# wwood/CoverM

Measured on AMD Instinct MI355X. Metric: aligned reads/s through coverm contig (mean trimmed_mean covered_fraction variance), higher is better.
Workload: dtype i32 depth / u64 sums / f32 estimators

## Files before the change

### coverm_amd/csrc/covermhip.hip

```cpp
#include "pileup_kernels.hip.h"
#include "prep_lean.hip.h"
#include "genome_kernels.hip.h"
#include "sep_kernels.hip.h"
#include "ingest_kernels.hip.h"
#include "group_kernels.hip.h"
#include "sam_kernels.hip.h"
#include "gene_kernels.hip.h"
#include "depth_kernels.hip.h"
#include "depth_bins_kernels.hip.h"
#include "depth_regions_kernels.hip.h"

#include <algorithm>
#include <atomic>
#include <cstddef>
#include <chrono>
#include <cstdio>
#include <dlfcn.h>
#include <functional>
#include <sched.h>
#include <cstdlib>
#include <cstring>
#include <map>
#include <mutex>
#include <string>
// ... 185 lines not shown
        if (why == Reset::SAM_FILE) return;
        feed = ingplan::FeedState{}; launched = 0; copy_cleared = -1;
        key_lo = 0; key_hi = ingplan::KEY_END; search_first = false; open_end = false;
        span_lo = 0; tail_key = ~0ull;
        s_alloc = 0; for (double &x : s_part) x = 0;
        stats = cov_ingest_stats{};
    }
};

struct cov_session {
    cov_config cfg{};
    hipStream_t stream = nullptr;
    std::string err;
    int tile = 1024;
    bool use_fast = true;
    int chunk_tiles = 4;
    int prep_kernel = 0;
    int est_lanes = -1;
    int fast_tables = 1;
    int n_cus = 256;

    uint32_t n_targets = 0;
    std::vector<uint32_t> h_tlen;
    std::vector<uint32_t> h_tile_first;
    uint32_t n_tiles = 0;
    DevBuf<u32> d_tlen, d_tile_contig, d_tile_start;
    DevBuf<u32> d_tile_first, d_tcnt, d_fov, d_tscan, d_ttop;
    DevBuf<u32> d_slow_list;
    uint32_t tile_shift = 10;
    DevBuf<u32> d_cx_list, d_cx_cnt, d_cx_cur, d_cx_scan, d_cx_top;
    DevBuf<uint2> d_cx_runs;
    DevBuf<DevContig> d_ctg_scratch;
    DevBuf<int32_t> d_depth_all; DevBuf<u64> d_depth_off; bool depth_all_valid = false;
    DevBuf<DevInterval> d_iv; DevBuf<DevIntervalStats> d_ivst; DevBuf<unsigned long long> d_ivhist; uint64_t ivhist_total = 0;
    DevBuf<uint8_t> gr_code; DevBuf<u32> gr_mism, gr_trec, gr_pprim, gr_tids; DevBuf<int32_t> gr_ttid, gr_tpos; DevBuf<double> gr_ident, gr_tident, gr_ck;
    DevBuf<u64> gr_bcnt, gr_bmism, gr_pmism, gr_glob; DevBuf<gnrc::Interval> gr_iv; DevBuf<covgn::Out> gr_out; DevBuf<covgn::Bounds> gr_bounds;
    float gene_ms = 0.f; uint32_t gene_launches = 0;
    struct DepthRuns {
        DevBuf<int32_t> arena; DevBuf<u32> woff, mask, rank, sums, run_off; DevBuf<u64> doff, total; DevBuf<dprc::Run> runs;
        std::vector<u32> h_woff, h_run_off;
        u64 chunk_bases = dprc::DEFAULT_CHUNK_BASES;
        bool valid = false;
        u32 lo = 0, next = 0, launches = 0;
// ... 238 lines not shown
int pileup_occupancy(const cov_session *s, std::atomic<int> (&occ_dev)[64], const void *kern, size_t smem) {
    std::atomic<int> &occ_slot = occ_dev[(unsigned)s->cfg.device & 63u];
    int occ = occ_slot.load(std::memory_order_relaxed);
    if (!occ) {
        (void)hipFuncSetAttribute(kern, hipFuncAttributeMaxDynamicSharedMemorySize, (int)smem);
        int nb = 0;
        if (hipOccupancyMaxActiveBlocksPerMultiprocessor(&nb, kern, 256, smem) != hipSuccess || nb < 1) {
            (void)hipGetLastError();
            nb = (int)std::max<size_t>(1, std::min<size_t>(8, (160 * 1024) / smem));
        }
        occ = nb; occ_slot.store(nb, std::memory_order_relaxed);
    }
    return occ;
}
u32 pileup_grid(const cov_session *s, int occ, u32 n_tiles) {
    const u32 n_chunks = (n_tiles + (u32)s->chunk_tiles - 1) / (u32)s->chunk_tiles, wg_per_cu = 8u * (u32)occ;
    return std::max(1u, std::min((n_chunks + 3) / 4, (u32)s->n_cus * wg_per_cu));
}

template <bool H, int TABLES>
void launch_fast_v(cov_session *s, const PileupArgs &a, u32 n_tiles) {
    const auto kern = TABLES == 1 ? &k_pileup_fast<H> : &k_pileup_fast2t<H>;
    const size_t smem = pileup_fast_smem_bytes(H, TABLES == 1 ? FAST_HB : FAST_HB7, TABLES);
    static std::atomic<int> occ_dev[64];
    const int occ = pileup_occupancy(s, occ_dev, reinterpret_cast<const void *>(kern), smem);
    hipLaunchKernelGGL(kern, dim3(pileup_grid(s, occ, n_tiles)), dim3(256), smem, s->stream, a, n_tiles, (u32)s->chunk_tiles);
}
template <bool H>
void launch_fast_t(cov_session *s, const PileupArgs &a, u32 n_tiles) {
    if (s->fast_tables == 2) launch_fast_v<H, 2>(s, a, n_tiles);
    else launch_fast_v<H, 1>(s, a, n_tiles);
}

template <bool H, bool W>
void launch_stream_t(cov_session *s, const PileupArgs &a, u32 n_tiles, bool slow_list_only = false) {
    const size_t smem = pileup_stream_smem_bytes();
    static std::atomic<int> occ_dev[64];
    const int occ = pileup_occupancy(s, occ_dev, reinterpret_cast<const void *>(&k_pileup_stream<H, W>), smem);
    if (slow_list_only) {
        hipLaunchKernelGGL((k_pileup_stream<H, W>), dim3((u32)s->n_cus), dim3(256), smem, s->stream, a, 0u, 1u,
                           (const u32 *)s->d_slow_list.p, (const u32 *)&s->d_glob.p->n_slow);
// ... 110 lines not shown
        const char *mode = getenv("COVERM_PILEUP");
        if (mode && !strcmp(mode, "stream")) s->use_fast = false;
        s->tile = STREAM_TW;
        stamp("hipSetDevice");
        int cus = 0;
        if (hipDeviceGetAttribute(&cus, hipDeviceAttributeMultiprocessorCount, cfg->device) == hipSuccess && cus > 0) s->n_cus = cus;
        stamp("device attribute");
    }
    if (cfg->want & COV_WANT_INGEST) s->ing.prep = std::async(std::launch::async, [s] { return ingest_prepare_(s); });
    if (const char *el = getenv("COVERM_EST_LANES")) s->est_lanes = atoi(el) ? 1 : 0;
    if (const char *ft = getenv("COVERM_FAST_TABLES")) s->fast_tables = atoi(ft) == 2 ? 2 : 1;
    if (const char *pk = getenv("COVERM_PREP_KERNEL")) s->prep_kernel = atoi(pk) == 7 ? 7 : 0;
    if (const char *im = getenv("COVERM_IDENTITY")) s->id_mode = strcmp(im, "serial") ? 1 : 0;
    { long long v; if (covknob::get("store_cap_records", v) && v >= 1) s->cap_records = std::min<uint64_t>((uint64_t)v, 0xfffffff0ull); }
    { long long v; if (covknob::get("store_cap_cigar", v) && v >= 1) s->cap_cigar = std::min<uint64_t>((uint64_t)v, 0xfffffff0ull); }
    { long long v; if (covknob::get("pileup_chunk_tiles", v) && v >= 1 && v <= 64) s->chunk_tiles = (int)v; }
    { long long v; if (covknob::get("depth_chunk_bases", v) && v >= 4) s->dr.chunk_bases = (uint64_t)v; }
    e = hipEventCreateWithFlags(&s->ev_prep_done, hipEventDisableTiming);
    if (e == hipSuccess) e = hipEventCreateWithFlags(&s->ev_side_done, hipEventDisableTiming);
    if (e == hipSuccess) e = hipStreamCreateWithFlags(&s->stream, hipStreamNonBlocking);
    if (e != hipSuccess) { g_create_error = std::string("hipStreamCreate: ") + hipGetErrorString(e); (void)ingest_prep_wait(s); delete s; return COV_ERR_HIP; }
    stamp("streams and events");
    e = bind_result_block(s, 1);
    if (e != hipSuccess) { g_create_error = std::string("hipMalloc: ") + hipGetErrorString(e); cov_destroy(s); return COV_ERR_HIP; }
    stamp("first hipMalloc");
    *out = s;
    return COV_OK;
}

static void ingest_free_buffers(cov_session *s) {
    s->ing.free_buffers();
    for (auto &b : s->m_text) b.release();
    s->m_nl.release(); s->m_tab.release(); s->m_line_end.release(); s->m_cnt.release(); s->m_rec_idx.release(); s->m_cig_idx.release();
}

void cov_destroy(cov_session *s) {
    if (!s) return;
    (void)ingest_prep_wait(s);
    (void)hipSetDevice(s->cfg.device);
    if (s->stream) (void)hipStreamSynchronize(s->stream);
    s->d_tlen.release(); s->d_tile_contig.release(); s->d_tile_start.release(); s->d_mask.release();
    s->d_grow.release(); s->d_gtids.release(); s->d_gseg_genome.release(); s->d_gseg_start.release(); s->d_genomes.release(); s->d_ghist.release(); s->d_ghist_top.release(); s->d_order.release();
    s->d_sgid.release(); s->d_sblk.release(); s->d_sent_pos.release(); s->d_stop_last1.release(); s->d_stop_first.release(); s->d_scounts.release(); s->d_scode.release();
    s->d_stop_cnt.release(); s->d_stop_seg.release(); s->d_sent.release();
    s->d_gout.release(); if (s->h_gout) (void)hipHostFree(s->h_gout); s->h_gout = nullptr;
    s->d_tile_first.release(); s->d_tcnt.release(); s->d_fov.release(); s->d_tscan.release(); s->d_ttop.release(); s->d_slow_list.release();
    s->dr.release(); s->d_ctg_scratch.release(); s->d_depth_all.release(); s->d_depth_off.release(); s->d_iv.release(); s->d_ivst.release(); s->d_ivhist.release();
    s->gr_code.release(); s->gr_mism.release(); s->gr_trec.release(); s->gr_pprim.release(); s->gr_tids.release(); s->gr_ttid.release(); s->gr_tpos.release(); s->gr_ident.release();
    s->gr_tident.release(); s->gr_ck.release(); s->gr_bcnt.release(); s->gr_bmism.release(); s->gr_pmism.release(); s->gr_glob.release(); s->gr_iv.release(); s->gr_out.release(); s->gr_bounds.release();
    s->d_cx_list.release(); s->d_cx_cnt.release(); s->d_cx_cur.release(); s->d_cx_scan.release(); s->d_cx_top.release(); s->d_cx_runs.release();
    if (s->side) {
        (void)hipStreamSynchronize(s->side);
        if (s->side_owned) (void)hipStreamDestroy(s->side);
        s->side = nullptr; s->side_owned = false;
    }
    s->ing.destroy();
    for (hipEvent_t e : s->sam_buf_free) if (e) (void)hipEventDestroy(e);
    for (hipEvent_t e : s->sam_ev) if (e) (void)hipEventDestroy(e);
    for (auto &b : s->m_text) b.release();
    s->m_blob.release(); s->m_nl.release(); s->m_tab.release(); s->m_res.release(); s->m_noff.release(); s->m_line_end.release(); s->m_cnt.release();
    s->m_rec_idx.release(); s->m_cig_idx.release(); s->m_slots.release(); for (auto &b : s->m_bsum) b.release();
// ... 38 lines not shown
    s->h_tile_first[n_targets] = (uint32_t)nt;
    s->n_tiles = (uint32_t)nt;
    std::vector<u32> tc(nt), ts(nt);
    for (uint32_t c = 0; c < n_targets; c++) {
        u32 k = s->h_tile_first[c];
        for (uint64_t p = 0; p < target_len[c]; p += (uint64_t)s->tile, k++) { tc[k] = c; ts[k] = (u32)p; }
    }
    HIPCHK(s->d_tlen.reserve(std::max<size_t>(1, n_targets), s->stream));
    HIPCHK(s->d_tile_contig.reserve(std::max<size_t>(1, nt), s->stream));
    HIPCHK(s->d_tile_start.reserve(std::max<size_t>(1, nt), s->stream));
    HIPCHK(s->d_desc.reserve(std::max<size_t>(2, 2 * nt), s->stream));
    HIPCHK(s->d_tile_first.reserve((size_t)n_targets + 1, s->stream));
    HIPCHK(s->d_tcnt.reserve(std::max<size_t>(1, nt), s->stream)); HIPCHK(s->d_fov.reserve(std::max<size_t>(1, nt), s->stream));
    HIPCHK(s->d_tscan.reserve(std::max<size_t>(1, nt), s->stream)); HIPCHK(s->d_ttop.reserve(nt / 1024 + 2, s->stream));
    HIPCHK(s->d_slow_list.reserve(std::max<size_t>(1, nt), s->stream));
    HIPCHK(s->d_cx_cnt.reserve(std::max<size_t>(1, nt), s->stream)); HIPCHK(s->d_cx_cur.reserve(std::max<size_t>(1, nt), s->stream));
    HIPCHK(s->d_cx_scan.reserve(std::max<size_t>(1, nt), s->stream)); HIPCHK(s->d_cx_top.reserve(nt / 1024 + 2, s->stream));
    HIPCHK(hipMemcpyAsync(s->d_tile_first.p, s->h_tile_first.data(), ((size_t)n_targets + 1) * 4, hipMemcpyHostToDevice, s->stream));
    s->tile_shift = 0;
    while ((1u << s->tile_shift) < (uint32_t)s->tile) s->tile_shift++;
    HIPCHK(bind_result_block(s, n_targets));
    if (n_targets) HIPCHK(hipMemcpyAsync(s->d_tlen.p, s->h_tlen.data(), (size_t)n_targets * 4, hipMemcpyHostToDevice, s->stream));
    if (nt) {
        HIPCHK(hipMemcpyAsync(s->d_tile_contig.p, tc.data(), nt * 4, hipMemcpyHostToDevice, s->stream));
        HIPCHK(hipMemcpyAsync(s->d_tile_start.p, ts.data(), nt * 4, hipMemcpyHostToDevice, s->stream));
    }
    HIPCHK(hipStreamSynchronize(s->stream));
    s->have_mask = false;
    genomes_off(s);
    s->finished = false;
// ... 427 lines not shown
    s->ev_fresh = -1;
    return COV_OK;
}

static cov_status stage_ranges(cov_session *s, const FinishPlan &p, const PassViews &v) {
    time_begin(s, COV_K_RANGES);
    const u32 n_blocks = (s->n_tiles + 1023u) / 1024u;
    const u32 cx_grid = (u32)s->n_cus * 8u;
    ScanPair sp{};
    sp.cnt[0] = s->d_tcnt.p; sp.scan[0] = s->d_tscan.p; sp.top[0] = s->d_ttop.p; sp.total[0] = nullptr;
    sp.cnt[1] = s->d_cx_cnt.p; sp.scan[1] = s->d_cx_scan.p; sp.top[1] = s->d_cx_top.p; sp.total[1] = &s->d_glob.p->cx_total;
    hipLaunchKernelGGL(k_tile_scan1, dim3(2u * n_blocks), dim3(1024), 0, v.st, sp, s->n_tiles, n_blocks);
    hipLaunchKernelGGL(k_tile_scan2, dim3(2), dim3(1024), 0, v.st, sp, n_blocks);
    hipLaunchKernelGGL((k_cx_expand<true>), dim3(cx_grid), dim3(256), 0, v.st, v.r, s->d_tlen.p, s->d_glob.p, v.cx, v.ti);
    u32 *slow_list = s->use_fast ? s->d_slow_list.p : nullptr;
    const auto ranges = p.want_hist ? &k_ranges<true> : &k_ranges<false>;
    hipLaunchKernelGGL(ranges, dim3((s->n_tiles + 255) / 256), dim3(256), 0, v.st, s->d_tile_contig.p, s->d_tile_start.p, s->n_tiles, s->d_tlen.p,
                       v.mask, s->d_ctg.p, s->d_desc.p, v.ti, s->d_tscan.p, s->d_ttop.p, v.cx, s->d_glob.p, slow_list);
    time_end(s, COV_K_RANGES);
    HIPCHK(hipGetLastError());
    return COV_OK;
}

static cov_status stage_hist_layout(cov_session *s, const PassViews &v) {
    time_begin(s, COV_K_HIST);
    const u32 hb = (v.nT + 1023u) / 1024u;
    HIPCHK(s->d_hist_top.reserve(hb, v.st));
    hipLaunchKernelGGL((k_hist_sum<0>), dim3(hb), dim3(1024), 0, v.st, (const DevContig *)s->d_ctg.p, v.nT, s->d_tlen.p, v.mask, v.excl, s->d_hist_top.p);
    hipLaunchKernelGGL((k_hist_off<0>), dim3(hb), dim3(1024), 0, v.st, s->d_ctg.p, v.nT, s->d_tlen.p, v.mask, v.excl, (const u64 *)s->d_hist_top.p, s->d_glob.p);
    hipLaunchKernelGGL(k_zero_u32, dim3(2048), dim3(256), 0, v.st, s->d_arena.p, &s->d_glob.p->hist_cap_total);
    time_end(s, COV_K_HIST);
    HIPCHK(hipGetLastError());
    return COV_OK;
// ... 1872 lines not shown
        return COV_OK;
    }
    if (ms_total) *ms_total = s->k_ms[k];
    if (launches) *launches = s->k_launches[k];
    return COV_OK;
}

cov_status cov_last_paths(const cov_session *s, cov_path_counts *out) {
    if (!s || !out) return COV_ERR_INVALID_ARG;
    out->listed_steps = s->h_glob.n_gen; out->generic_only = s->last_gen_all ? 1u : 0u;
    out->slow_tiles = s->h_glob.n_slow; out->bucket_records = s->h_glob.n_cx;
    out->bucket_entries = (uint32_t)std::min<uint64_t>(s->h_glob.cx_total, 0xffffffffull); out->passes = s->last_passes;
    return COV_OK;
}

cov_status cov_copy_run_words(const cov_session *cs, uint64_t *out) {
    cov_session *s = const_cast<cov_session *>(cs);
    if (!s || !s->finished) return COV_ERR_STATE;
    if (s->spill.active || s->adopted || s->store.n_records == 0 || s->d_runs.cap < s->store.n_records) return COV_ERR_STATE;
    if (!out) return COV_ERR_INVALID_ARG;
    static_assert(sizeof(uint2) == sizeof(uint64_t), "a run word is eight bytes, x first");
    HIPCHK(hipSetDevice(s->cfg.device));
    HIPCHK(hipMemcpyAsync(out, s->d_runs.p, (size_t)s->store.n_records * sizeof(uint2), hipMemcpyDeviceToHost, s->stream));
    HIPCHK(hipStreamSynchronize(s->stream));
    return COV_OK;
}

uint32_t cov_store_spills(const cov_session *s) { return s ? s->spill.count : 0u; }

cov_status cov_set_estimators(cov_session *s, const cov_estimator *est, uint32_t n_est) {
// ... 186 lines not shown
```

### coverm_amd/csrc/pileup_kernels.hip.h

```cpp
#pragma once
#include <hip/hip_runtime.h>
#include <stdint.h>

#define HSTC_FN __host__ __device__ __forceinline__
#include "hist_stats_core.h"
#include "scan_ops.hip.h"

namespace covk {

typedef unsigned long long u64;
typedef unsigned int u32;

constexpr u32 F_POS_UNSORTED = 1u;
constexpr u32 RW_SINGLE = 0u, RW_DOUBLE = 1u, RW_COMPLEX = 2u, RW_BUCKET = 3u;
constexpr u32 FAST_MAX_CAND = 8191u;
constexpr u32 TILE_F_GENERIC = 1u, TILE_F_SLOW = 2u;
constexpr u32 CX_MIN_OPS = 16;

struct DevContig {
    u64 n_primary, n_pass, n_nonsupp, sum_nm, sum_indel;
    double id_primary, id_nonsupp;
    u64 sum_d, sum_d2, cov_win, cov_full, proc_win;
    u64 hist_off;
    u32 first_rec, last_rec;
    u32 rec_start, rec_end;
    u32 n_groups;
    u32 max_span;
    u32 flags;
    u32 hist_cap;
    u32 min_d, max_d;
    u32 hist_len;
// ... 3 lines not shown
static_assert(sizeof(DevContig) == 160, "DevContig layout");

constexpr u32 COUNTER_SLOTS = 64;
struct DevGlobal {
    u64 first_error;
    u64 hist_cap_total;
    u64 chist_total;
    u32 internal_error;
    u32 n_cx;
    u64 cx_total;
    u32 n_slow;
    u32 n_gen;
    u64 pad2[2];
    u64 prim_slots[COUNTER_SLOTS * 8];
    u64 cons_slots[COUNTER_SLOTS * 8];
    u32 pad_q[8 * 16];
};

struct FilterCfg {
    u32 include_improper_pairs, include_supplementary, include_secondary;
    u32 filter_single, min_mapq, min_aligned_length;
    float min_percent_identity, min_aligned_percent;
};

struct Records {
    const int32_t *tid, *pos;
    const uint16_t *flag;
    const uint8_t *mapq;
    const u32 *nm;
    const uint8_t *nm_kind;
    const u32 *l_seq;
// ... 52 lines not shown
    double *identp, *identn;
    u32 n, cigar_end, n_targets, shift, steps;
    u32 gate_mask;
    u32 p1_mask;
    u32 min_mapq, min_aligned_length;
    float min_percent_identity, min_aligned_percent;
};
struct PrepArgs { PrepHot hot; PrepCold cold; };

__global__ void k_init(DevContig *ctg, u32 n_targets, DevGlobal *g, TileIdx ti, CxIdx cx, PrepArgs *pa_out, PrepArgs pa) {
    u32 c = blockIdx.x * blockDim.x + threadIdx.x;
    if (c == 0 && pa_out != nullptr) *pa_out = pa;
    if (c < ti.n_tiles) { ti.tcnt[c] = 0u; ti.fov[c] = 0xffffffffu; cx.cnt[c] = 0u; cx.cur[c] = 0u; }
    if (c == 0) {
        g->first_error = ~0ull; g->hist_cap_total = 0; g->chist_total = 0; g->internal_error = 0;
        g->n_cx = 0; g->cx_total = 0; g->n_slow = 0; g->n_gen = 0;
    }
    if (c < COUNTER_SLOTS * 8) { g->prim_slots[c] = 0; g->cons_slots[c] = 0; }
    if (c >= n_targets) return;
    DevContig z;
    z.n_primary = z.n_pass = z.n_nonsupp = z.sum_nm = z.sum_indel = 0;
    z.id_primary = z.id_nonsupp = 0.0;
    z.sum_d = z.sum_d2 = z.cov_win = z.cov_full = z.proc_win = 0;
    z.hist_off = 0;
    z.first_rec = 0xffffffffu; z.last_rec = 0;
    z.rec_start = 0xffffffffu; z.rec_end = 0;
    z.n_groups = 0; z.max_span = 0; z.flags = 0; z.hist_cap = 0;
    z.min_d = 0xffffffffu; z.max_d = 0; z.hist_len = 0; z.cov_out = 0; z.chist_off = 0;
    ctg[c] = z;
}

// ... 579 lines not shown
__global__ __launch_bounds__(256) void k_cx_expand(Records r, const u32 *__restrict__ tlen, DevGlobal *g, CxIdx cx, TileIdx ti) {
    cx_expand_body<FILL>(r, tlen, g, cx, ti, blockIdx.x * 4u + (threadIdx.x >> 6), gridDim.x * 4u);
}

__global__ __launch_bounds__(256) void k_post_prep(Records r, const u32 *__restrict__ tlen, DevGlobal *g, CxIdx cx, TileIdx ti, DevContig *ctg, u32 n_targets,
                                                   const PrepPartial *__restrict__ part, u32 n_parts, u32 chunk_recs, u32 n_red) {
    if (blockIdx.x < n_red) prep_reduce_body(blockIdx.x * 4u + (threadIdx.x >> 6), ctg, n_targets, part, n_parts, chunk_recs);
    else cx_expand_body<false>(r, tlen, g, cx, ti, (blockIdx.x - n_red) * 4u + (threadIdx.x >> 6), (gridDim.x - n_red) * 4u);
}

template <bool WANT_HIST>
__global__ __launch_bounds__(256) void k_ranges(const u32 *__restrict__ tile_contig, const u32 *__restrict__ tile_start,
                                                u32 n_tiles, const u32 *__restrict__ tlen, const uint8_t *__restrict__ mask,
                                                DevContig *ctg, uint4 *__restrict__ desc, TileIdx ti,
                                                const u32 *__restrict__ tscan, const u32 *__restrict__ ttop, CxIdx cx,
                                                DevGlobal *__restrict__ g, u32 *__restrict__ slow_list) {
    const u32 t = blockIdx.x * blockDim.x + threadIdx.x;
    if (t >= n_tiles) return;
    const u32 c = tile_contig[t];
    DevContig *C = &ctg[c];
    uint4 out = make_uint4(0u, 0u, tlen[c], 0u);
    u32 cxn = 0, cxo = 0;
    if (C->n_pass != 0 && (mask == nullptr || mask[c])) {
        const u32 rs = C->rec_start, re = C->rec_end;
        cxn = g->cx_total <= cx.runs_cap ? cx.cnt[t] : 0u;
        cxo = cx.cscan[t] + cx.ctop[t >> 10];
        if (C->n_groups != 1u) out.w = 1u;
        if (C->n_groups != 1u || (C->flags & F_POS_UNSORTED)) {
            out.x = rs; out.y = re;
        } else {
            const u32 tf = ti.tile_first[c];
            const u32 before = (tscan[t] + ttop[t >> 10]) - (tscan[tf] + ttop[tf >> 10]);
            const u32 f = rs + before;
            out.y = min(f + ti.tcnt[t], re);
            out.x = max(min(f, ti.fov[t]), rs);
            out.x = min(out.x, out.y);
        }
    }
    if (out.x < out.y || cxn) {
        if (out.w || out.y - out.x + cxn > FAST_MAX_CAND) {
            out.w |= TILE_F_SLOW;
            if (slow_list != nullptr) slow_list[atomicAdd(&g->n_slow, 1u)] = t;
        }
    }
    if (WANT_HIST) {
        const u32 npass = (u32)min(C->n_pass, (u64)0xffffffffu);
        const u32 cap = min(out.y - out.x + cxn, npass);
        if (__all(c == (u32)__builtin_amdgcn_readfirstlane((int)c))) {
            const u32 m = wave_max_u32(cap);
            if (lane_id() == 0 && m) atomicMax(&C->hist_cap, m);
        } else if (cap) atomicMax(&C->hist_cap, cap);
    }
    desc[2 * t] = out;
    desc[2 * t + 1] = make_uint4(c, tile_start[t], cxo, cxn);
}

template <int MODE>
// ... 558 lines not shown
    }
}

constexpr size_t pileup_stream_smem_bytes() { return (size_t)4 * ((size_t)STREAM_TW * 4 + STREAM_HB * 4); }

constexpr int FAST_TW = 1024, FAST_HB = 512;
constexpr int FAST_HB7 = 384;
constexpr size_t pileup_fast_smem_bytes(bool hist, int hb = FAST_HB, int tables = 2) { return (size_t)4 * ((size_t)FAST_TW * 2 * tables + (hist ? (size_t)hb * 4 : 0)); }

typedef short v2i16 __attribute__((ext_vector_type(2)));
typedef __attribute__((address_space(3))) u32 lds_u32_t;
__device__ __forceinline__ u32 lds_addr_of(const u32 *p) { return (u32)(uintptr_t)(lds_u32_t *)p; }
__device__ __forceinline__ void lds_atomic_add(u32 addr, u32 x) { (void)__hip_atomic_fetch_add((lds_u32_t *)(uintptr_t)addr, x, __ATOMIC_RELAXED, __HIP_MEMORY_SCOPE_WORKGROUP); }

template <bool WANT_HIST, int HB, int TABLES>
__device__ __forceinline__ void pileup_fast_body(const PileupArgs &a, u32 n_tiles, u32 chunk_tiles) {
    constexpr int TW = FAST_TW, HBW = HB;
    constexpr int DS = TABLES == 1 ? 2 : 0;
    constexpr size_t WB = (size_t)TW * 2 * TABLES + (WANT_HIST ? (size_t)HBW * 4 : 0);
    extern __shared__ __attribute__((aligned(16))) char smem[];
    const int lane = threadIdx.x & 63, w = threadIdx.x >> 6;
    u32 *S = reinterpret_cast<u32 *>(smem + (size_t)w * WB);
    u32 *E = TABLES == 2 ? S + TW / 2 : S;
    u32 *lhist = S + (TW / 2) * TABLES;
    uint4 *S4 = reinterpret_cast<uint4 *>(S), *E4 = reinterpret_cast<uint4 *>(E);
    const u32 wave_id = (u32)__builtin_amdgcn_readfirstlane((int)(blockIdx.x * 4u + (u32)w)), n_waves = gridDim.x * 4u;
    if (WANT_HIST) {
#pragma unroll
        for (int b = lane; b < HBW; b += 64) lhist[b] = 0u;
    }
    u64 sum_d = 0, sum_d2 = 0, proc_win = 0;
    u32 cov_w = 0, cov_f = 0, mn = 0xffffffffu, mx = 0;
    u32 cov_o = 0;
    int cur_c = -1;
    u64 hoff = 0; u32 hcap = 0;
    const u64 excl = a.excl;
    u32 hbound = 0;
    auto drain = [&]() {
        lds_fence();
        for (u32 b = (u32)lane; b <= hbound; b += 64) {
            const u32 x = lhist[b];
// ... 32 lines not shown
                if (c2) atomicAdd(&C->cov_full, (u64)c2);
                if (proc_win) {
                    atomicAdd(&C->proc_win, proc_win);
                    atomicMin(&C->min_d, m1);
                    atomicMax(&C->max_d, m2);
                }
            }
        }
        sum_d = sum_d2 = 0; proc_win = 0; cov_w = cov_f = 0; mn = 0xffffffffu; mx = 0;
    };
    auto load_runs = [&](const uint4 &d, uint2 &r0, uint2 &r1) {
        const u32 i0 = d.x + (u32)lane, i1 = i0 + 64u;
        r0 = i0 < d.y ? a.runs[i0] : make_uint2(0u, 0u);
        r1 = i1 < d.y ? a.runs[i1] : make_uint2(0u, 0u);
    };
    const u32 n_chunks = (n_tiles + chunk_tiles - 1) / chunk_tiles;
    if (wave_id >= n_chunks) return;
    u32 ch = wave_id;
    u32 t = ch * chunk_tiles, t_end = min(t + chunk_tiles, n_tiles);
    uint4 ds = a.desc[2 * (size_t)(a.tile_base + t)], dC1 = a.desc[2 * (size_t)(a.tile_base + t) + 1];
    uint2 rw0, rw1;
    load_runs(ds, rw0, rw1);
    for (;;) {
        u32 tn = t + 1, tn_end = t_end, chn = ch;
        bool chunk_end = false;
        if (tn >= t_end) {
            chunk_end = true;
            chn = ch + n_waves;
            tn = chn < n_chunks ? chn * chunk_tiles : 0xffffffffu;
            tn_end = chn < n_chunks ? min(tn + chunk_tiles, n_tiles) : 0u;
        }
        const bool have_next = tn != 0xffffffffu;
        uint4 nds = make_uint4(0u, 0u, 0u, 0u), ndC1 = make_uint4(0u, 0u, 0u, 0u);
        if (have_next) { nds = a.desc[2 * (size_t)(a.tile_base + tn)]; ndC1 = a.desc[2 * (size_t)(a.tile_base + tn) + 1]; }

        const u32 c = dC1.x, lo = dC1.y, L = ds.z, cxo = dC1.z, cxn = dC1.w;
        const bool live = (ds.x < ds.y || cxn != 0u) && !(ds.w & TILE_F_SLOW);
        uint4 sv0, sv1, ev0, ev1;
        if (live) {
            if ((int)c != cur_c) {
                flush();
                cur_c = (int)c;
                if (WANT_HIST) { hoff = a.ctg[c].hist_off; hcap = a.ctg[c].hist_cap; }
            }
            const u32 zb = TABLES == 2 ? 0u : 0x80008000u;
            const uint4 z4 = make_uint4(zb, zb, zb, zb);
            S4[2 * lane] = z4; S4[2 * lane + 1] = z4;
            if (TABLES == 2) { E4[2 * lane] = z4; E4[2 * lane + 1] = z4; }
            asm volatile("" ::: "memory");
            const u32 hi = lo + TW;
            auto add_run = [&](u32 s, u32 e) {
                if (s < hi && e > lo) {
// ... 133 lines not shown
                    const u32 p = p0 + (u32)j;
                    const bool in_w = win_any && p >= wst && p < wet;
                    d += dj;
                    const u32 du = (u32)d >> DS;
                    if (p < L) cov_f += du != 0u ? 1u : 0u;
                    if (in_w) {
                        sum_d += du; sum_d2 += (u64)du * du;
                        cov_w += du != 0u ? 1u : 0u;
                        mn = min(mn, du); mx = max(mx, du);
                    }
                }
            }
        }
        if (chunk_end) { flush(); cur_c = -1; }
        if (!have_next) break;
        t = tn; t_end = tn_end; ch = chn; ds = nds; dC1 = ndC1; rw0 = nrw0; rw1 = nrw1;
    }
}

template <bool WANT_HIST>
__global__ __launch_bounds__(256) __attribute__((amdgpu_waves_per_eu(7, 7))) void k_pileup_fast(PileupArgs a, u32 n_tiles, u32 chunk_tiles) {
    pileup_fast_body<WANT_HIST, FAST_HB, 1>(a, n_tiles, chunk_tiles);
}
template <bool WANT_HIST>
__global__ __launch_bounds__(256) __attribute__((amdgpu_waves_per_eu(6, 6))) void k_pileup_fast2t(PileupArgs a, u32 n_tiles, u32 chunk_tiles) {
    pileup_fast_body<WANT_HIST, FAST_HB7, 2>(a, n_tiles, chunk_tiles);
}


struct DevEstimator { int kind; float min_frac; u64 excl; int exclude_mismatches; float trim_min, trim_max; u32 pad; };
static_assert(sizeof(DevEstimator) == 32, "DevEstimator mirrors cov_estimator");
constexpr u32 EST_MAX = 16;
struct EstParams { DevEstimator e[EST_MAX]; u32 n; u32 pad; };
enum { EST_MEAN = 0, EST_TRIMMED_MEAN = 1, EST_PILEUP_COUNTS = 2, EST_COVERED_FRACTION = 3, EST_COVERED_BASES = 4, EST_RPKM = 5, EST_TPM = 6,
       EST_VARIANCE = 7, EST_LENGTH = 8, EST_READ_COUNT = 9, EST_READS_PER_BASE = 10, EST_ANIR = 11 };

__device__ __forceinline__ float est_f32(u64 x) { return __ull2float_rn(x); }
__device__ __forceinline__ u64 est_f32_to_usize(float x) {
    if (!(x == x) || x <= 0.0f) return 0ull;
    if (x >= 18446744073709551616.0f) return ~0ull;
    return (u64)x;
// ... 295 lines not shown
```

### coverm_amd/engine.py

```python
import ctypes as C
from dataclasses import dataclass
from typing import Optional

import numpy as np

from . import native
from .native import CovBatch, CovConfig, CovError, CovSummary


@dataclass
class RecordBatch:
    tid: np.ndarray
    pos: np.ndarray
    flag: np.ndarray
    mapq: np.ndarray
    nm: np.ndarray
    nm_kind: np.ndarray
    l_seq: np.ndarray
    cigar_off: np.ndarray
    cigar: np.ndarray

    @property
    def n_records(self):
        return int(self.tid.shape[0])
# ... 354 lines not shown
    def kernel_ms(self):
        out = {}
        for k, name in native.KERNEL_NAMES.items():
            ms = C.c_double(0)
            n = C.c_uint32(0)
            self._check(self._lib.cov_kernel_ms(self._h, k, C.byref(ms), C.byref(n)))
            out[name] = (ms.value, n.value)
        return out

    def last_paths(self):
        v = (C.c_uint32 * 6)()
        self._check(self._lib.cov_last_paths(self._h, C.byref(v)))
        return dict(listed_steps=int(v[0]), generic_only=bool(v[1]), slow_tiles=int(v[2]), bucket_records=int(v[3]),
                    bucket_entries=int(v[4]), passes=int(v[5]))

    def run_words(self):
        n = C.c_uint64(0)
        self._check(self._lib.cov_copy_records(self._h, None, C.byref(n), None))
        out = np.zeros(max(1, int(n.value)), dtype=np.uint64)
        self._check(self._lib.cov_copy_run_words(self._h, out.ctypes.data_as(C.c_void_p)))
        return out[:int(n.value)]

    def algorithmic_bytes(self):
        b = C.c_uint64(0)
        self._check(self._lib.cov_algorithmic_bytes(self._h, C.byref(b)))
        return int(b.value)
```

### coverm_amd/native.py

```python
import ctypes as C
import os

import numpy as np

_HERE = os.path.dirname(os.path.abspath(__file__))
LIB_PATH = os.path.join(_HERE, "libcovermhip.so")

COV_OK = 0
ERR_UNSORTED, ERR_NM_MISSING, ERR_NM_BADTYPE, ERR_POS_OOB, ERR_BAD_CIGAR, ERR_BAD_TID = 1, 2, 3, 4, 6, 7
ERR_INVALID_ARG, ERR_HIP, ERR_STATE = 16, 17, 18
WANT_HIST, WANT_IDENTITY = 1, 2
WANT_IDENTITY_PRIMARY_ONLY, WANT_IDENTITY_NONSUPP_ONLY = 4, 8
K_PREP, K_RANGES, K_PILEUP, K_IDENTITY, K_HIST, K_HIST_COMPACT, K_ESTIMATE, K_COUNT = 0, 1, 2, 3, 4, 5, 6, 15
K_GENOME = 7
K_GROUP = 8
K_SEP = 10
K_GENE_READS = 11
K_DEPTH_RUNS = 12
K_DEPTH_BINS = 13
K_DEPTH_REGIONS = 14
K_SAM = 9
KERNEL_NAMES = {K_PREP: "k_prep", K_RANGES: "k_ranges", K_PILEUP: "k_pileup", K_IDENTITY: "k_identity",
                K_HIST: "k_hist", K_HIST_COMPACT: "k_hist_compact", K_ESTIMATE: "k_estimate"}

# ... 51 lines not shown
    _fields_ = [("arena_bases", C.c_uint64), ("n_bins", C.c_uint64), ("arena_ms", C.c_double), ("bins_ms", C.c_double),
                ("tid_lo", C.c_uint32), ("tid_next", C.c_uint32), ("bin_size", C.c_uint32), ("reserved", C.c_uint32)]


DEPTH_REGION_DTYPE = np.dtype([("tid", "<u4"), ("start", "<u4"), ("end", "<u4"), ("reserved", "<u4")])
assert DEPTH_REGION_DTYPE.itemsize == 16


class CovDepthRegionsInfo(C.Structure):
    _fields_ = [("arena_bases", C.c_uint64), ("n_regions", C.c_uint64), ("n_pieces", C.c_uint64), ("arena_ms", C.c_double), ("regions_ms", C.c_double),
                ("tid_lo", C.c_uint32), ("tid_next", C.c_uint32)]


EXPORTS = ["cov_abi_version", "cov_create", "cov_destroy", "cov_last_error", "cov_set_targets",
           "cov_set_target_mask", "cov_push_batch", "cov_push_batch_device", "cov_finish", "cov_fetch_hist",
           "cov_copy_depth", "cov_reset", "cov_kernel_ms", "cov_algorithmic_bytes", "cov_last_paths", "cov_copy_run_words",
           "cov_set_genomes", "cov_finish_genomes", "cov_fetch_genome_estimates", "cov_fetch_genome_stats",
           "cov_set_genome_runs", "cov_genome_entry_count", "cov_fetch_genome_entries",
           "cov_sam_begin", "cov_sam_window_bytes", "cov_sam_slot_wait", "cov_sam_feed", "cov_sam_end", "cov_ingest_last_stats",
           "cov_interval_reads_compute", "cov_depth_runs_compute", "cov_depth_runs_fetch", "cov_depth_runs_last",
           "cov_depth_bins_compute", "cov_depth_bins_fetch", "cov_depth_bins_last",
           "cov_depth_regions_set", "cov_depth_regions_compute", "cov_depth_regions_fetch", "cov_depth_regions_last"]

_lib = None


class NativeLibraryMissing(RuntimeError):
    pass


def _torch_hip_first():
# ... 23 lines not shown
    L.cov_last_error.argtypes = [C.c_void_p]
    L.cov_create.argtypes = [C.POINTER(CovConfig), C.POINTER(C.c_void_p)]
    L.cov_destroy.argtypes = [C.c_void_p]
    L.cov_destroy.restype = None
    L.cov_set_targets.argtypes = [C.c_void_p, C.c_uint32, C.c_void_p]
    L.cov_set_target_mask.argtypes = [C.c_void_p, C.c_void_p]
    L.cov_push_batch.argtypes = [C.c_void_p, C.POINTER(CovBatch)]
    L.cov_push_batch_device.argtypes = [C.c_void_p, C.POINTER(CovBatch)]
    L.cov_finish.argtypes = [C.c_void_p, C.c_void_p, C.POINTER(CovSummary)]
    L.cov_fetch_hist.argtypes = [C.c_void_p, C.c_void_p]
    L.cov_copy_depth.argtypes = [C.c_void_p, C.c_uint32, C.c_void_p]
    L.cov_reset.argtypes = [C.c_void_p]
    L.cov_kernel_ms.argtypes = [C.c_void_p, C.c_int, C.POINTER(C.c_double), C.POINTER(C.c_uint32)]
    L.cov_algorithmic_bytes.argtypes = [C.c_void_p, C.POINTER(C.c_uint64)]
    L.cov_last_paths.argtypes = [C.c_void_p, C.POINTER(C.c_uint32 * 6)]
    L.cov_copy_run_words.argtypes = [C.c_void_p, C.c_void_p]
    L.cov_copy_records.argtypes = [C.c_void_p, C.c_void_p, C.POINTER(C.c_uint64), C.POINTER(C.c_uint64)]
    L.cov_set_estimators.argtypes = [C.c_void_p, C.c_void_p, C.c_uint32]
    L.cov_fetch_estimates.argtypes = [C.c_void_p, C.c_void_p]
    L.cov_set_genomes.argtypes = [C.c_void_p, C.c_void_p, C.c_uint32]
    L.cov_finish_genomes.argtypes = [C.c_void_p, C.POINTER(CovSummary)]
    L.cov_fetch_genome_estimates.argtypes = [C.c_void_p, C.c_void_p]
    L.cov_fetch_genome_stats.argtypes = [C.c_void_p, C.c_void_p]
    L.cov_set_genome_runs.argtypes = [C.c_void_p, C.c_void_p, C.c_uint32]
    L.cov_genome_entry_count.argtypes = [C.c_void_p, C.POINTER(C.c_uint32)]
    L.cov_fetch_genome_entries.argtypes = [C.c_void_p, C.c_void_p]
    L.cov_store_spills.argtypes = [C.c_void_p]
    L.cov_store_spills.restype = C.c_uint32
    L.cov_group_records.argtypes = [C.c_void_p, C.POINTER(C.c_uint64)]
    L.cov_ingest_want_grouping.argtypes = [C.c_void_p, C.c_int]
# ... 21 lines not shown
```

### include/covermhip.h

```cpp
#ifndef COVERMHIP_H
#define COVERMHIP_H

#include <stddef.h>
#include <stdint.h>

#ifdef __cplusplus
extern "C" {
#endif

#define COVERMHIP_ABI_VERSION 1

typedef struct cov_session cov_session;

typedef enum {
    COV_OK = 0,
    COV_ERR_UNSORTED = 1,
    COV_ERR_NM_MISSING = 2,
    COV_ERR_NM_BADTYPE = 3,
    COV_ERR_POS_OOB = 4,
    COV_ERR_BAD_CIGAR = 6,
    COV_ERR_BAD_TID = 7,
    COV_ERR_INVALID_ARG = 16,
    COV_ERR_HIP = 17,
    COV_ERR_STATE = 18,
// ... 141 lines not shown
    float min_percent_identity_pair, min_aligned_percent_pair;
} cov_pair_filter;
cov_status cov_ingest_want_mates(cov_session *s, int on);
cov_status cov_pair_filter_apply(cov_session *s, const cov_pair_filter *f, uint64_t *n_selected, uint64_t *n_primary);
cov_status cov_ingest_want_grouping(cov_session *s, int on);
cov_status cov_group_records(cov_session *s, uint64_t *n_moved);
cov_status cov_copy_records(cov_session *s, const cov_batch *host, uint64_t *n_records, uint64_t *n_cigar);
cov_status cov_copy_mates(cov_session *s, int32_t *mtid, uint64_t *qh1, uint32_t *qh2);

cov_status cov_gather(cov_session *const *sessions, uint32_t n, uint32_t root);
cov_status cov_gathered(cov_session *root_session, uint32_t rank, cov_contig_stats *stats, cov_summary *summary);

cov_status cov_kernel_ms(const cov_session *s, cov_kernel_id k, double *ms_total, uint32_t *launches);
typedef struct { uint32_t listed_steps, generic_only, slow_tiles, bucket_records, bucket_entries, passes; } cov_path_counts;
cov_status cov_last_paths(const cov_session *s, cov_path_counts *out);
cov_status cov_copy_run_words(const cov_session *s, uint64_t *out);
cov_status cov_algorithmic_bytes(const cov_session *s, uint64_t *bytes);

typedef struct {
    int32_t kind;
    float min_fraction_covered_bases;
    uint64_t contig_end_exclusion;
    int32_t exclude_mismatches;
    float trim_min, trim_max;
} cov_estimator;
#define COV_EST_MEAN 0
#define COV_EST_TRIMMED_MEAN 1
#define COV_EST_PILEUP_COUNTS 2
#define COV_EST_COVERED_FRACTION 3
#define COV_EST_COVERED_BASES 4
// ... 102 lines not shown
```

Measured before the change: 49.89 billion.

## Schedule deep pileup tiles first via device list and shrink fast-pileup workgroups to one wave

The ranges kernel now flags tiles whose candidate count exceeds a threshold as deep and appends them to a device-side list using a wave ballot and atomic. The fast pileup kernel visits those deep tiles first, one tile per visit, and then walks the remaining chunks while skipping deep tiles, which is meant to reduce load imbalance from heavy tiles landing at the end. Workgroups are shrunk to a single wave with shared memory scaled to match, the grid cap is recomputed through a shared schedule header, and waves_per_eu for the single-table kernel changes from 7 to 8. The cost is an extra atomic pass and list buffer, plus less locality for listed tiles because each visit changes contig.

```diff
diff --git a/coverm_amd/csrc/covermhip.hip b/coverm_amd/csrc/covermhip.hip
--- a/coverm_amd/csrc/covermhip.hip
+++ b/coverm_amd/csrc/covermhip.hip
@@ -223,7 +223,8 @@
     std::string err;
     int tile = 1024;
     bool use_fast = true;
-    int chunk_tiles = 4;
+    int chunk_tiles = (int)psched::CHUNK_TILES;
+    int chunk_tiles_listed = (int)psched::CHUNK_TILES_LISTED;
     int prep_kernel = 0;
     int est_lanes = -1;
     int fast_tables = 1;
@@ -236,6 +237,9 @@
     DevBuf<u32> d_tlen, d_tile_contig, d_tile_start;
     DevBuf<u32> d_tile_first, d_tcnt, d_fov, d_tscan, d_ttop;
     DevBuf<u32> d_slow_list;
+    DevBuf<u32> d_deep_list;
+    uint32_t deep_min = psched::DEEP_MIN;
+    uint32_t last_pileup_waves = 0, last_pileup_chunk = 0;
     uint32_t tile_shift = 10;
     DevBuf<u32> d_cx_list, d_cx_cnt, d_cx_cur, d_cx_scan, d_cx_top;
     DevBuf<uint2> d_cx_runs;
@@ -504,9 +508,9 @@
     return occ;
 }
 u32 pileup_grid(const cov_session *s, int occ, u32 n_tiles) {
-    const u32 n_chunks = (n_tiles + (u32)s->chunk_tiles - 1) / (u32)s->chunk_tiles, wg_per_cu = 8u * (u32)occ;
-    return std::max(1u, std::min((n_chunks + 3) / 4, (u32)s->n_cus * wg_per_cu));
-}
+    return psched::grid_of(n_tiles, (u32)s->chunk_tiles, (u32)s->n_cus, (u32)occ * 4u, psched::STREAM_WG_WAVES);
+}
+const u32 *pileup_deep_list(const cov_session *s) { return s->use_fast && s->deep_min != 0u ? s->d_deep_list.p : nullptr; }
 
 template <bool H, int TABLES>
 void launch_fast_v(cov_session *s, const PileupArgs &a, u32 n_tiles) {
@@ -514,7 +518,12 @@
     const size_t smem = pileup_fast_smem_bytes(H, TABLES == 1 ? FAST_HB : FAST_HB7, TABLES);
     static std::atomic<int> occ_dev[64];
     const int occ = pileup_occupancy(s, occ_dev, reinterpret_cast<const void *>(kern), smem);
-    hipLaunchKernelGGL(kern, dim3(pileup_grid(s, occ, n_tiles)), dim3(256), smem, s->stream, a, n_tiles, (u32)s->chunk_tiles);
+    const u32 *deep_list = a.tile_base == 0u && n_tiles == s->n_tiles ? pileup_deep_list(s) : nullptr;
+    const u32 chunk = (u32)(deep_list != nullptr ? s->chunk_tiles_listed : s->chunk_tiles);
+    constexpr u32 WGW = psched::FAST_WG_WAVES;
+    const u32 grid = psched::grid_of(n_tiles, chunk, (u32)s->n_cus, (u32)occ * 4u, WGW);
+    s->last_pileup_waves = grid * WGW; s->last_pileup_chunk = chunk;
+    hipLaunchKernelGGL(kern, dim3(grid), dim3(64u * WGW), smem / 4u * WGW, s->stream, a, n_tiles, chunk, deep_list, (const u32 *)&s->d_glob.p->n_deep);
 }
 template <bool H>
 void launch_fast_t(cov_session *s, const PileupArgs &a, u32 n_tiles) {
@@ -655,7 +664,8 @@
     if (const char *im = getenv("COVERM_IDENTITY")) s->id_mode = strcmp(im, "serial") ? 1 : 0;
     { long long v; if (covknob::get("store_cap_records", v) && v >= 1) s->cap_records = std::min<uint64_t>((uint64_t)v, 0xfffffff0ull); }
     { long long v; if (covknob::get("store_cap_cigar", v) && v >= 1) s->cap_cigar = std::min<uint64_t>((uint64_t)v, 0xfffffff0ull); }
-    { long long v; if (covknob::get("pileup_chunk_tiles", v) && v >= 1 && v <= 64) s->chunk_tiles = (int)v; }
+    { long long v; if (covknob::get("pileup_chunk_tiles", v) && v >= 1 && v <= 64) s->chunk_tiles = s->chunk_tiles_listed = (int)v; }
+    { long long v; if (covknob::get("pileup_deep_min", v) && v >= 0 && v <= 0x7fffffffll) s->deep_min = (uint32_t)v; }
     { long long v; if (covknob::get("depth_chunk_bases", v) && v >= 4) s->dr.chunk_bases = (uint64_t)v; }
     e = hipEventCreateWithFlags(&s->ev_prep_done, hipEventDisableTiming);
     if (e == hipSuccess) e = hipEventCreateWithFlags(&s->ev_side_done, hipEventDisableTiming);
@@ -685,7 +695,7 @@
     s->d_sgid.release(); s->d_sblk.release(); s->d_sent_pos.release(); s->d_stop_last1.release(); s->d_stop_first.release(); s->d_scounts.release(); s->d_scode.release();
     s->d_stop_cnt.release(); s->d_stop_seg.release(); s->d_sent.release();
     s->d_gout.release(); if (s->h_gout) (void)hipHostFree(s->h_gout); s->h_gout = nullptr;
-    s->d_tile_first.release(); s->d_tcnt.release(); s->d_fov.release(); s->d_tscan.release(); s->d_ttop.release(); s->d_slow_list.release();
+    s->d_tile_first.release(); s->d_tcnt.release(); s->d_fov.release(); s->d_tscan.release(); s->d_ttop.release(); s->d_slow_list.release(); s->d_deep_list.release();
     s->dr.release(); s->d_ctg_scratch.release(); s->d_depth_all.release(); s->d_depth_off.release(); s->d_iv.release(); s->d_ivst.release(); s->d_ivhist.release();
     s->gr_code.release(); s->gr_mism.release(); s->gr_trec.release(); s->gr_pprim.release(); s->gr_tids.release(); s->gr_ttid.release(); s->gr_tpos.release(); s->gr_ident.release();
     s->gr_tident.release(); s->gr_ck.release(); s->gr_bcnt.release(); s->gr_bmism.release(); s->gr_pmism.release(); s->gr_glob.release(); s->gr_iv.release(); s->gr_out.release(); s->gr_bounds.release();
@@ -754,6 +764,7 @@
     HIPCHK(s->d_tcnt.reserve(std::max<size_t>(1, nt), s->stream)); HIPCHK(s->d_fov.reserve(std::max<size_t>(1, nt), s->stream));
     HIPCHK(s->d_tscan.reserve(std::max<size_t>(1, nt), s->stream)); HIPCHK(s->d_ttop.reserve(nt / 1024 + 2, s->stream));
     HIPCHK(s->d_slow_list.reserve(std::max<size_t>(1, nt), s->stream));
+    HIPCHK(s->d_deep_list.reserve(std::max<size_t>(1, nt), s->stream));
     HIPCHK(s->d_cx_cnt.reserve(std::max<size_t>(1, nt), s->stream)); HIPCHK(s->d_cx_cur.reserve(std::max<size_t>(1, nt), s->stream));
     HIPCHK(s->d_cx_scan.reserve(std::max<size_t>(1, nt), s->stream)); HIPCHK(s->d_cx_top.reserve(nt / 1024 + 2, s->stream));
     HIPCHK(hipMemcpyAsync(s->d_tile_first.p, s->h_tile_first.data(), ((size_t)n_targets + 1) * 4, hipMemcpyHostToDevice, s->stream));
@@ -1211,9 +1222,10 @@
     hipLaunchKernelGGL(k_tile_scan2, dim3(2), dim3(1024), 0, v.st, sp, n_blocks);
     hipLaunchKernelGGL((k_cx_expand<true>), dim3(cx_grid), dim3(256), 0, v.st, v.r, s->d_tlen.p, s->d_glob.p, v.cx, v.ti);
     u32 *slow_list = s->use_fast ? s->d_slow_list.p : nullptr;
+    u32 *deep_list = const_cast<u32 *>(pileup_deep_list(s));
     const auto ranges = p.want_hist ? &k_ranges<true> : &k_ranges<false>;
     hipLaunchKernelGGL(ranges, dim3((s->n_tiles + 255) / 256), dim3(256), 0, v.st, s->d_tile_contig.p, s->d_tile_start.p, s->n_tiles, s->d_tlen.p,
-                       v.mask, s->d_ctg.p, s->d_desc.p, v.ti, s->d_tscan.p, s->d_ttop.p, v.cx, s->d_glob.p, slow_list);
+                       v.mask, s->d_ctg.p, s->d_desc.p, v.ti, s->d_tscan.p, s->d_ttop.p, v.cx, s->d_glob.p, slow_list, deep_list, s->deep_min);
     time_end(s, COV_K_RANGES);
     HIPCHK(hipGetLastError());
     return COV_OK;
@@ -3116,6 +3128,12 @@
     return COV_OK;
 }
 
+cov_status cov_pileup_schedule(const cov_session *s, uint32_t out[4]) {
+    if (!s || !out) return COV_ERR_INVALID_ARG;
+    out[0] = s->h_glob.n_deep; out[1] = s->last_pileup_waves; out[2] = s->last_pileup_chunk; out[3] = s->deep_min;
+    return COV_OK;
+}
+
 cov_status cov_copy_run_words(const cov_session *cs, uint64_t *out) {
     cov_session *s = const_cast<cov_session *>(cs);
     if (!s || !s->finished) return COV_ERR_STATE;
diff --git a/coverm_amd/csrc/pileup_kernels.hip.h b/coverm_amd/csrc/pileup_kernels.hip.h
--- a/coverm_amd/csrc/pileup_kernels.hip.h
+++ b/coverm_amd/csrc/pileup_kernels.hip.h
@@ -4,6 +4,8 @@
 
 #define HSTC_FN __host__ __device__ __forceinline__
 #include "hist_stats_core.h"
+#define PSCHED_FN __host__ __device__ __forceinline__
+#include "pileup_schedule_core.h"
 #include "scan_ops.hip.h"
 
 namespace covk {
@@ -14,7 +16,7 @@
 constexpr u32 F_POS_UNSORTED = 1u;
 constexpr u32 RW_SINGLE = 0u, RW_DOUBLE = 1u, RW_COMPLEX = 2u, RW_BUCKET = 3u;
 constexpr u32 FAST_MAX_CAND = 8191u;
-constexpr u32 TILE_F_GENERIC = 1u, TILE_F_SLOW = 2u;
+constexpr u32 TILE_F_GENERIC = 1u, TILE_F_SLOW = 2u, TILE_F_DEEP = 4u;
 constexpr u32 CX_MIN_OPS = 16;
 
 struct DevContig {
@@ -48,7 +50,8 @@
     u64 pad2[2];
     u64 prim_slots[COUNTER_SLOTS * 8];
     u64 cons_slots[COUNTER_SLOTS * 8];
-    u32 pad_q[8 * 16];
+    u32 n_deep;
+    u32 pad_q[8 * 16 - 1];
 };
 
 struct FilterCfg {
@@ -131,7 +134,7 @@
     if (c < ti.n_tiles) { ti.tcnt[c] = 0u; ti.fov[c] = 0xffffffffu; cx.cnt[c] = 0u; cx.cur[c] = 0u; }
     if (c == 0) {
         g->first_error = ~0ull; g->hist_cap_total = 0; g->chist_total = 0; g->internal_error = 0;
-        g->n_cx = 0; g->cx_total = 0; g->n_slow = 0; g->n_gen = 0;
+        g->n_cx = 0; g->cx_total = 0; g->n_slow = 0; g->n_gen = 0; g->n_deep = 0;
     }
     if (c < COUNTER_SLOTS * 8) { g->prim_slots[c] = 0; g->cons_slots[c] = 0; }
     if (c >= n_targets) return;
@@ -741,7 +744,7 @@
                                                 u32 n_tiles, const u32 *__restrict__ tlen, const uint8_t *__restrict__ mask,
                                                 DevContig *ctg, uint4 *__restrict__ desc, TileIdx ti,
                                                 const u32 *__restrict__ tscan, const u32 *__restrict__ ttop, CxIdx cx,
-                                                DevGlobal *__restrict__ g, u32 *__restrict__ slow_list) {
+                                                DevGlobal *__restrict__ g, u32 *__restrict__ slow_list, u32 *__restrict__ deep_list, u32 deep_min) {
     const u32 t = blockIdx.x * blockDim.x + threadIdx.x;
     if (t >= n_tiles) return;
     const u32 c = tile_contig[t];
@@ -768,6 +771,20 @@
         if (out.w || out.y - out.x + cxn > FAST_MAX_CAND) {
             out.w |= TILE_F_SLOW;
             if (slow_list != nullptr) slow_list[atomicAdd(&g->n_slow, 1u)] = t;
+        }
+    }
+    if (deep_list != nullptr) {
+        const bool deep = (out.x < out.y || cxn) && !(out.w & TILE_F_SLOW) && out.y - out.x + cxn >= deep_min;
+        const u64 dm = __ballot(deep);
+        if (dm != 0ull) {
+            const int lane = lane_id(), lead = __ffsll((long long)dm) - 1;
+            u32 base = 0;
+            if (lane == lead) base = atomicAdd(&g->n_deep, (u32)__popcll(dm));
+            base = (u32)__builtin_amdgcn_readlane((int)base, lead);
+            if (deep) {
+                out.w |= TILE_F_DEEP;
+                deep_list[base + (u32)__popcll(dm & (lane == 0 ? 0ull : (~0ull >> (64 - lane))))] = t;
+            }
         }
     }
     if (WANT_HIST) {
@@ -1356,7 +1373,7 @@
 __device__ __forceinline__ void lds_atomic_add(u32 addr, u32 x) { (void)__hip_atomic_fetch_add((lds_u32_t *)(uintptr_t)addr, x, __ATOMIC_RELAXED, __HIP_MEMORY_SCOPE_WORKGROUP); }
 
 template <bool WANT_HIST, int HB, int TABLES>
-__device__ __forceinline__ void pileup_fast_body(const PileupArgs &a, u32 n_tiles, u32 chunk_tiles) {
+__device__ __forceinline__ void pileup_fast_body(const PileupArgs &a, u32 n_tiles, u32 chunk_tiles, const u32 *__restrict__ deep_list, const u32 *__restrict__ n_deep_ptr) {
     constexpr int TW = FAST_TW, HBW = HB;
     constexpr int DS = TABLES == 1 ? 2 : 0;
     constexpr size_t WB = (size_t)TW * 2 * TABLES + (WANT_HIST ? (size_t)HBW * 4 : 0);
@@ -1366,7 +1383,8 @@
     u32 *E = TABLES == 2 ? S + TW / 2 : S;
     u32 *lhist = S + (TW / 2) * TABLES;
     uint4 *S4 = reinterpret_cast<uint4 *>(S), *E4 = reinterpret_cast<uint4 *>(E);
-    const u32 wave_id = (u32)__builtin_amdgcn_readfirstlane((int)(blockIdx.x * 4u + (u32)w)), n_waves = gridDim.x * 4u;
+    const u32 wpb = blockDim.x >> 6;
+    const u32 wave_id = (u32)__builtin_amdgcn_readfirstlane((int)(blockIdx.x * wpb + (u32)w)), n_waves = gridDim.x * wpb;
     if (WANT_HIST) {
 #pragma unroll
         for (int b = lane; b < HBW; b += 64) lhist[b] = 0u;
@@ -1429,28 +1447,38 @@
         r0 = i0 < d.y ? a.runs[i0] : make_uint2(0u, 0u);
         r1 = i1 < d.y ? a.runs[i1] : make_uint2(0u, 0u);
     };
-    const u32 n_chunks = (n_tiles + chunk_tiles - 1) / chunk_tiles;
-    if (wave_id >= n_chunks) return;
-    u32 ch = wave_id;
-    u32 t = ch * chunk_tiles, t_end = min(t + chunk_tiles, n_tiles);
+    const psched::Launch sched = psched::launch_of(n_tiles, chunk_tiles, n_waves, deep_list != nullptr ? *n_deep_ptr : 0u);
+    const u32 skip_flags = TILE_F_SLOW | (deep_list != nullptr ? TILE_F_DEEP : 0u);
+    psched::Visit vis = psched::first(sched, wave_id);
+    if (vis.done) return;
+    u32 lt_next = 0;
+    u32 t, t_end;
+    if (vis.in_list) {
+        t = deep_list[vis.idx]; t_end = t + 1u;
+        if (vis.idx + n_waves < sched.n_deep) lt_next = deep_list[vis.idx + n_waves];
+    } else { t = psched::chunk_t0(sched, vis.idx); t_end = psched::chunk_t1(sched, vis.idx); }
     uint4 ds = a.desc[2 * (size_t)(a.tile_base + t)], dC1 = a.desc[2 * (size_t)(a.tile_base + t) + 1];
     uint2 rw0, rw1;
     load_runs(ds, rw0, rw1);
     for (;;) {
-        u32 tn = t + 1, tn_end = t_end, chn = ch;
+        u32 tn = t + 1, tn_end = t_end;
+        psched::Visit visn = vis;
         bool chunk_end = false;
         if (tn >= t_end) {
             chunk_end = true;
-            chn = ch + n_waves;
-            tn = chn < n_chunks ? chn * chunk_tiles : 0xffffffffu;
-            tn_end = chn < n_chunks ? min(tn + chunk_tiles, n_tiles) : 0u;
+            visn = psched::next(sched, wave_id, vis);
+            if (visn.done) { tn = 0xffffffffu; tn_end = 0u; }
+            else if (visn.in_list) {
+                tn = lt_next; tn_end = tn + 1u;
+                if (visn.idx + n_waves < sched.n_deep) lt_next = deep_list[visn.idx + n_waves];
+            } else { tn = psched::chunk_t0(sched, visn.idx); tn_end = psched::chunk_t1(sched, visn.idx); }
         }
         const bool have_next = tn != 0xffffffffu;
         uint4 nds = make_uint4(0u, 0u, 0u, 0u), ndC1 = make_uint4(0u, 0u, 0u, 0u);
         if (have_next) { nds = a.desc[2 * (size_t)(a.tile_base + tn)]; ndC1 = a.desc[2 * (size_t)(a.tile_base + tn) + 1]; }
 
         const u32 c = dC1.x, lo = dC1.y, L = ds.z, cxo = dC1.z, cxn = dC1.w;
-        const bool live = (ds.x < ds.y || cxn != 0u) && !(ds.w & TILE_F_SLOW);
+        const bool live = (ds.x < ds.y || cxn != 0u) && (vis.in_list || !(ds.w & skip_flags));
         uint4 sv0, sv1, ev0, ev1;
         if (live) {
             if ((int)c != cur_c) {
@@ -1614,17 +1642,17 @@
         }
         if (chunk_end) { flush(); cur_c = -1; }
         if (!have_next) break;
-        t = tn; t_end = tn_end; ch = chn; ds = nds; dC1 = ndC1; rw0 = nrw0; rw1 = nrw1;
+        t = tn; t_end = tn_end; vis = visn; ds = nds; dC1 = ndC1; rw0 = nrw0; rw1 = nrw1;
     }
 }
 
 template <bool WANT_HIST>
-__global__ __launch_bounds__(256) __attribute__((amdgpu_waves_per_eu(7, 7))) void k_pileup_fast(PileupArgs a, u32 n_tiles, u32 chunk_tiles) {
-    pileup_fast_body<WANT_HIST, FAST_HB, 1>(a, n_tiles, chunk_tiles);
+__global__ __launch_bounds__(256) __attribute__((amdgpu_waves_per_eu(8, 8))) void k_pileup_fast(PileupArgs a, u32 n_tiles, u32 chunk_tiles, const u32 *__restrict__ deep_list, const u32 *__restrict__ n_deep) {
+    pileup_fast_body<WANT_HIST, FAST_HB, 1>(a, n_tiles, chunk_tiles, deep_list, n_deep);
 }
 template <bool WANT_HIST>
-__global__ __launch_bounds__(256) __attribute__((amdgpu_waves_per_eu(6, 6))) void k_pileup_fast2t(PileupArgs a, u32 n_tiles, u32 chunk_tiles) {
-    pileup_fast_body<WANT_HIST, FAST_HB7, 2>(a, n_tiles, chunk_tiles);
+__global__ __launch_bounds__(256) __attribute__((amdgpu_waves_per_eu(6, 6))) void k_pileup_fast2t(PileupArgs a, u32 n_tiles, u32 chunk_tiles, const u32 *__restrict__ deep_list, const u32 *__restrict__ n_deep) {
+    pileup_fast_body<WANT_HIST, FAST_HB7, 2>(a, n_tiles, chunk_tiles, deep_list, n_deep);
 }
 
 
diff --git a/coverm_amd/csrc/pileup_schedule_core.h b/coverm_amd/csrc/pileup_schedule_core.h
--- /dev/null
+++ b/coverm_amd/csrc/pileup_schedule_core.h
@@ -0,0 +1,49 @@
+#pragma once
+#include <stdint.h>
+
+#ifndef PSCHED_FN
+#define PSCHED_FN inline
+#endif
+
+namespace psched {
+
+typedef unsigned int u32;
+
+constexpr u32 PILEUP_ROUNDS = 8u;
+constexpr u32 FAST_WG_WAVES = 1u, STREAM_WG_WAVES = 4u;
+constexpr u32 CHUNK_TILES = 4u, CHUNK_TILES_LISTED = 8u;
+constexpr u32 DEEP_MIN = 192u;
+PSCHED_FN u32 n_chunks_of(u32 n_tiles, u32 chunk_tiles) { return n_tiles / chunk_tiles + (n_tiles % chunk_tiles != 0u ? 1u : 0u); }
+PSCHED_FN u32 grid_of(u32 n_tiles, u32 chunk_tiles, u32 n_cus, u32 waves_per_cu, u32 wg_waves) {
+    const u32 nc = n_chunks_of(n_tiles, chunk_tiles), need = nc / wg_waves + (nc % wg_waves != 0u ? 1u : 0u), cap = n_cus * (waves_per_cu / wg_waves) * PILEUP_ROUNDS;
+    const u32 g = need < cap ? need : cap;
+    return g > 0u ? g : 1u;
+}
+
+struct Launch { u32 n_tiles, chunk_tiles, n_waves, n_deep, n_chunks; };
+PSCHED_FN Launch launch_of(u32 n_tiles, u32 chunk_tiles, u32 n_waves, u32 n_deep) {
+    return Launch{n_tiles, chunk_tiles, n_waves, n_deep, n_chunks_of(n_tiles, chunk_tiles)};
+}
+
+struct Visit { u32 idx; bool in_list, done; };
+
+PSCHED_FN Visit first_chunk(const Launch &L, u32 wave) {
+    return Visit{wave, false, wave >= L.n_chunks};
+}
+PSCHED_FN Visit first(const Launch &L, u32 wave) {
+    if (wave < L.n_deep) return Visit{wave, true, false};
+    return first_chunk(L, wave);
+}
+PSCHED_FN Visit next(const Launch &L, u32 wave, const Visit &v) {
+    const u32 nx = v.idx + L.n_waves, end = v.in_list ? L.n_deep : L.n_chunks;
+    if (nx < end && nx >= v.idx) return Visit{nx, v.in_list, false};
+    if (v.in_list) return first_chunk(L, wave);
+    return Visit{0u, false, true};
+}
+PSCHED_FN u32 chunk_t0(const Launch &L, u32 ch) { return ch * L.chunk_tiles; }
+PSCHED_FN u32 chunk_t1(const Launch &L, u32 ch) {
+    const u32 t0 = ch * L.chunk_tiles;
+    return L.n_tiles - t0 < L.chunk_tiles ? L.n_tiles : t0 + L.chunk_tiles;
+}
+
+}
diff --git a/coverm_amd/engine.py b/coverm_amd/engine.py
--- a/coverm_amd/engine.py
+++ b/coverm_amd/engine.py
@@ -392,6 +392,11 @@
         return dict(listed_steps=int(v[0]), generic_only=bool(v[1]), slow_tiles=int(v[2]), bucket_records=int(v[3]),
                     bucket_entries=int(v[4]), passes=int(v[5]))
 
+    def pileup_schedule(self):
+        v = (C.c_uint32 * 4)()
+        self._check(self._lib.cov_pileup_schedule(self._h, C.byref(v)))
+        return dict(deep_tiles=int(v[0]), waves=int(v[1]), chunk_tiles=int(v[2]), deep_min=int(v[3]))
+
     def run_words(self):
         n = C.c_uint64(0)
         self._check(self._lib.cov_copy_records(self._h, None, C.byref(n), None))
diff --git a/coverm_amd/native.py b/coverm_amd/native.py
--- a/coverm_amd/native.py
+++ b/coverm_amd/native.py
@@ -89,7 +89,7 @@
 
 EXPORTS = ["cov_abi_version", "cov_create", "cov_destroy", "cov_last_error", "cov_set_targets",
            "cov_set_target_mask", "cov_push_batch", "cov_push_batch_device", "cov_finish", "cov_fetch_hist",
-           "cov_copy_depth", "cov_reset", "cov_kernel_ms", "cov_algorithmic_bytes", "cov_last_paths", "cov_copy_run_words",
+           "cov_copy_depth", "cov_reset", "cov_kernel_ms", "cov_algorithmic_bytes", "cov_last_paths", "cov_pileup_schedule", "cov_copy_run_words",
            "cov_set_genomes", "cov_finish_genomes", "cov_fetch_genome_estimates", "cov_fetch_genome_stats",
            "cov_set_genome_runs", "cov_genome_entry_count", "cov_fetch_genome_entries",
            "cov_sam_begin", "cov_sam_window_bytes", "cov_sam_slot_wait", "cov_sam_feed", "cov_sam_end", "cov_ingest_last_stats",
@@ -143,6 +143,7 @@
     L.cov_kernel_ms.argtypes = [C.c_void_p, C.c_int, C.POINTER(C.c_double), C.POINTER(C.c_uint32)]
     L.cov_algorithmic_bytes.argtypes = [C.c_void_p, C.POINTER(C.c_uint64)]
     L.cov_last_paths.argtypes = [C.c_void_p, C.POINTER(C.c_uint32 * 6)]
+    L.cov_pileup_schedule.argtypes = [C.c_void_p, C.POINTER(C.c_uint32 * 4)]
     L.cov_copy_run_words.argtypes = [C.c_void_p, C.c_void_p]
     L.cov_copy_records.argtypes = [C.c_void_p, C.c_void_p, C.POINTER(C.c_uint64), C.POINTER(C.c_uint64)]
     L.cov_set_estimators.argtypes = [C.c_void_p, C.c_void_p, C.c_uint32]
diff --git a/include/covermhip.h b/include/covermhip.h
--- a/include/covermhip.h
+++ b/include/covermhip.h
@@ -179,6 +179,7 @@
 cov_status cov_kernel_ms(const cov_session *s, cov_kernel_id k, double *ms_total, uint32_t *launches);
 typedef struct { uint32_t listed_steps, generic_only, slow_tiles, bucket_records, bucket_entries, passes; } cov_path_counts;
 cov_status cov_last_paths(const cov_session *s, cov_path_counts *out);
+cov_status cov_pileup_schedule(const cov_session *s, uint32_t out[4]);
 cov_status cov_copy_run_words(const cov_session *s, uint64_t *out);
 cov_status cov_algorithmic_bytes(const cov_session *s, uint64_t *bytes);
 
```

Result: faster. 51.14 billion (median of 6 runs) (+2.5%).
